# jacarvalho/mpd-public

Measured on AMD Instinct MI355X. Metric: denoising-steps/s, higher is better.
Workload: dtype f32; 1 GPU; cfg2: EnvDense2D-RobotPointMass shape, 100 trajectories (1 context(s)) x H=64 x D=4, T=100 (+5) reverse steps, unguided, U-Net dim_mults (1, 2, 4, 8), one plan = one bench step; parallelism=single, denoising_steps_per_plan=105

## Files before the change

### include/mpdx.h

```cpp
#ifndef MPDX_H
#define MPDX_H

#include <stddef.h>
#include <stdint.h>

#ifdef __cplusplus
extern "C" {
#endif

#define MPDX_E_INVALID   (-1)
#define MPDX_E_NOTFOUND  (-2)
#define MPDX_E_STATE     (-3)

#define MPDX_MAX_LEVELS 8

typedef struct mpdx_unet mpdx_unet;

typedef struct mpdx_unet_cfg {
    int32_t state_dim;
    int32_t n_support_points;
    int32_t unet_input_dim;
    int32_t n_levels;
    int32_t dim_mults[MPDX_MAX_LEVELS];
    int32_t time_emb_dim;
// ... 165 lines not shown
int mpdx_plan(mpdx_unet* u, const float* packed_dev, const float* timetab_dev, int T, const mpdx_step_coefs* coefs,
              int n_without_noise, float* x, const float* noise, const float* hard_start, const float* hard_goal,
              float* chain, int B, float* ws, const mpdx_guide_params* guide, int n_guide_steps, int t_start_guide,
              uint32_t* guide_flags, int n_per_ctx, uint64_t rng_seed, uint64_t rng_offset, void* stream);

int mpdx_unet_profile(mpdx_unet* u, const float* packed_dev, const float* timetab_dev, int T, const float* x, int t,
                      int B, float* ws, void* stream, int cap, float* ms_out, double* flops_out,
                      const char** names_out, int* n_out);
int mpdx_layer_trace(mpdx_unet* u, const float* packed_dev, const float* timetab_dev, const float* x, int layer, int B, float* ws,
                     void* stream, long long* stamps32);
int mpdx_fused_trace(mpdx_unet* u, const float* packed_dev, const float* timetab_dev, const float* x, int seg, int B,
                     float* ws, void* stream, long long* stamps_out, int cap, int* n_out, int* nops_out);
int mpdx_unet_time_units(mpdx_unet* u, const float* packed_dev, const float* timetab_dev, int T, const float* x, int t, int B,
                         float* ws, void* stream, int unit_first, int unit_last, int reps, float* ms_avg);
int mpdx_unet_time_without(mpdx_unet* u, const float* packed_dev, const float* timetab_dev, int T, const float* x, int t, int B,
                           float* ws, void* stream, unsigned long long skip_mask, int reps, float* ms_avg);
int mpdx_unet_unit_layer(const mpdx_unet* u, int B, int i);
int mpdx_unet_fused_program(const mpdx_unet* u, int seg);
double mpdx_unet_unit_bytes(const mpdx_unet* u, int B, int i);
int mpdx_unet_unit_is_pair(const mpdx_unet* u, int B, int i);
int mpdx_bench_layer(mpdx_unet* u, const float* packed_dev, const float* timetab_dev, const float* x, int layer, int B,
                     float* ws, void* stream, int reps, int dbg, float* ms_per_launch);
int mpdx_unet_layer_tile(const mpdx_unet* u, int i, int B, char* buf, size_t buflen);

#ifdef __cplusplus
}
#endif
#endif
```

### mpd_public_amd/_lib.py

```python
from __future__ import annotations

import ctypes as C
from pathlib import Path

import os as _os

_LIB_PATH = Path(_os.environ["MPDX_LIB"]) if _os.environ.get("MPDX_LIB") else Path(__file__).resolve().parent / "libmpdx.so"
_lib = None

MAX_LEVELS = 8


class UnetCfg(C.Structure):
    _fields_ = [("state_dim", C.c_int32), ("n_support_points", C.c_int32), ("unet_input_dim", C.c_int32),
                ("n_levels", C.c_int32), ("dim_mults", C.c_int32 * MAX_LEVELS), ("time_emb_dim", C.c_int32),
                ("self_attention", C.c_int32)]


class StepCoefs(C.Structure):
    _fields_ = [("sqrt_recip_alphas_cumprod", C.c_float), ("sqrt_recipm1_alphas_cumprod", C.c_float),
                ("posterior_mean_coef1", C.c_float), ("posterior_mean_coef2", C.c_float),
                ("noise_scale", C.c_float), ("noise_std_extra", C.c_float),
                ("predict_epsilon", C.c_int32), ("clip_denoised", C.c_int32), ("ddim_k1", C.c_float), ("ddim_k2", C.c_float),
                ("guide_scale", C.c_float)]
# ... 56 lines not shown
    "mpdx_weighted_loss": (_i, [_vp, _vp, _vp, _vp, _vp, _i, _vp, _i, _i, _i, _vp]),
    "mpdx_plan": (_i, [_vp, _vp, _vp, _i, C.POINTER(StepCoefs), _i, _vp, _vp, _vp, _vp, _vp, _i, _vp,
                        C.POINTER(GuideParams), _i, _i, _vp, _i, C.c_uint64, C.c_uint64, _vp]),
    "mpdx_guide_step": (_i, [C.POINTER(GuideParams), _vp, _vp, _vp, _vp, _vp, _vp, _i, _i, _i, _i, _vp]),
    "mpdx_guide_step_scaled": (_i, [C.POINTER(GuideParams), _vp, _vp, _vp, _vp, _vp, _vp, _i, _i, _i, _i, _f, _vp]),
    "mpdx_guide_time": (_i, [C.POINTER(GuideParams), _vp, _vp, _vp, _i, _i, _i, _i, _i, _vp, C.POINTER(C.c_float)]),
    "mpdx_traj_metrics": (_i, [C.POINTER(GuideParams), _vp, _vp, _i, _i, _i, _i, _vp]),
    "mpdx_traj_metrics_mask": (_i, [C.POINTER(GuideParams), _vp, _vp, _vp, _i, _i, _i, _i, _vp]),
    "mpdx_guide_trace": (_i, [C.POINTER(GuideParams), _vp, _vp, _i, _i, _i, _vp, C.POINTER(C.c_longlong)]),
    "mpdx_absmax": (_i, [_vp, _vp, _i, _i, _i, _i, _vp]),
    "mpdx_sdf_grid_bake": (_i, [C.POINTER(GuideParams), _i, _vp, _vp, C.POINTER(C.c_int * 3), C.POINTER(C.c_float * 3), _f, _vp]),
    "mpdx_unet_profile": (_i, [_vp, _vp, _vp, _i, _vp, _i, _i, _vp, _vp, _i, C.POINTER(C.c_float), C.POINTER(C.c_double),
                                C.POINTER(C.c_char_p), C.POINTER(C.c_int)]),
    "mpdx_layer_trace": (_i, [_vp, _vp, _vp, _vp, _i, _i, _vp, _vp, C.POINTER(C.c_longlong)]),
    "mpdx_fused_trace": (_i, [_vp, _vp, _vp, _vp, _i, _i, _vp, _vp, C.POINTER(C.c_longlong), _i, C.POINTER(C.c_int), C.POINTER(C.c_int)]),
    "mpdx_unet_time_units": (_i, [_vp, _vp, _vp, _i, _vp, _i, _i, _vp, _vp, _i, _i, _i, C.POINTER(C.c_float)]),
    "mpdx_unet_time_without": (_i, [_vp, _vp, _vp, _i, _vp, _i, _i, _vp, _vp, C.c_uint64, _i, C.POINTER(C.c_float)]),
    "mpdx_unet_unit_layer": (_i, [_vp, _i, _i]),
    "mpdx_unet_unit_is_pair": (_i, [_vp, _i, _i]),
    "mpdx_unet_unit_bytes": (C.c_double, [_vp, _i, _i]),
    "mpdx_unet_fused_program": (_i, [_vp, _i]),
    "mpdx_bench_layer": (_i, [_vp, _vp, _vp, _vp, _i, _i, _vp, _vp, _i, _i, C.POINTER(C.c_float)]),
    "mpdx_unet_layer_tile": (_i, [_vp, _i, _i, C.c_char_p, _sz]),
    "mpdx_randn": (_i, [_vp, _sz, C.c_uint64, C.c_uint64, _vp]),
    "mpdx_train_flat_floats": (_sz, [_vp]),
    "mpdx_train_dgrad_pack_floats": (_sz, [_vp]),
    "mpdx_train_workspace_floats": (_sz, [_vp, _i]),
    "mpdx_train_param_offset": (_i, [_vp, _i, C.POINTER(_sz), C.POINTER(_sz)]),
    "mpdx_train_pack": (_i, [_vp, _vp, _vp, _vp, _vp]),
    "mpdx_train_loss_backward": (_i, [_vp, _vp, _vp, _vp, _vp, _vp, _vp, _vp, _vp, _vp, _vp, _vp, _vp, _vp, _i, _i, _i, _i, _f, _vp, _vp, _vp]),
    "mpdx_adam_step": (_i, [_vp, _vp, _vp, _vp, _sz, _f, _f, _f, _f, _i, _f, _vp, _vp]),
    "mpdx_train_draw": (_i, [_vp, C.c_uint64, _vp]),
    "mpdx_ema_update": (_i, [_vp, _vp, _sz, _f, _vp]),
    "mpdx_gpmp_step": (_i, [C.POINTER(GuideParams), C.POINTER(GpmpOpts), _vp, _vp, _vp, _i, _i, _i, _i, _vp]),
    "mpdx_rrt_paths": (_i, [C.POINTER(GuideParams), _vp, _vp, _vp, _vp, _vp, _vp, _vp, _i, _i, _i, _f, _i, _i, _vp]),
    "mpdx_rrt_connect": (_i, [C.POINTER(GuideParams), C.POINTER(RrtOpts), _vp, _vp, _vp, _vp, _vp, _vp, _vp, _i, _vp]),
}


def lib_path() -> Path:
    return _LIB_PATH


class LibraryUnavailable(RuntimeError):
    """libmpdx.so is missing or cannot be loaded on this host (every compute entry point raises it; nothing falls back)"""

# ... 38 lines not shown
```

### mpd_public_amd/csrc/conv_block.hpp

```cpp
#pragma once
#include <hip/hip_runtime.h>
#include <stdint.h>

#include <type_traits>

#if defined(MPDX_LOOP_ABLATION) && !defined(MPDX_DEV_HOOKS)
#define MPDX_DEV_HOOKS 1
#endif
#ifdef MPDX_DEV_HOOKS
#define MPDX_TRACE_PTR(p) (p)
#define MPDX_DBG(a, bits) ((a).dbg & (bits))
#else
#define MPDX_TRACE_PTR(p) ((long long*)nullptr)
#define MPDX_DBG(a, bits) (0)
#endif

namespace mpdx {

typedef float f32x4 __attribute__((ext_vector_type(4)));
typedef float f32x2 __attribute__((ext_vector_type(2)));

enum : int { CONV_S1 = 0, CONV_DOWN = 1, CONV_UPT = 2 };
enum : int { EPI_BIAS = 0, EPI_GN_MISH = 1, EPI_GN_MISH_GEN = 2, EPI_GN_BWD = 3 };

// ... 99 lines not shown
    const float u2 = ((float)(c2 >> 8) + 0.5f) * (1.0f / 16777216.0f), u3 = ((float)(c3 >> 8) + 0.5f) * (1.0f / 16777216.0f);
    const float r0 = sqrtf(-2.0f * logf(u0)), r1 = sqrtf(-2.0f * logf(u2));
    float s0, cs0, s1, cs1;
    sincosf(6.28318530717958647692f * u1, &s0, &cs0);
    sincosf(6.28318530717958647692f * u3, &s1, &cs1);
    z[0] = r0 * cs0; z[1] = r0 * s0; z[2] = r1 * cs1; z[3] = r1 * s1;
}
__device__ __forceinline__ float philox_normal_at(uint64_t seed, uint64_t offset, uint64_t i) {
    float z[4];
    philox_normal4(seed, offset + (i >> 2), z);
    const int c = (int)(i & 3);
    return c == 0 ? z[0] : c == 1 ? z[1] : c == 2 ? z[2] : z[3];
}

template <int MODE, int KS>
struct ConvGeom {
    static constexpr int PAD = (MODE == CONV_S1) ? KS / 2 : 1;
    static constexpr int NTAP = (MODE == CONV_UPT) ? 2 : KS;
    static constexpr int NSLOT = (MODE == CONV_UPT) ? 4 : KS;
};

__host__ __device__ inline int upt_slot_to_k(int slot) { return slot == 0 ? 1 : slot == 1 ? 3 : slot == 2 ? 2 : 0; }

struct GeoAny { static constexpr int L = 0, NC16 = 0, RSPAD = 0; };
template <int NC16_> struct GeoL8 { static constexpr int L = 8, NC16 = NC16_, RSPAD = 8; };
template <int NC16_> struct GeoUp8 { static constexpr int L = 8, NC16 = NC16_, RSPAD = 4; };
constexpr int geo_ilog2(int v) { return v <= 1 ? 0 : 1 + geo_ilog2(v >> 1); }

template <int MODE, int KS, int EPI, int MT, int NT, int WN, int WK, class GEO = GeoAny, int TBRES = -1>
__device__ __forceinline__ void conv_block_body(const ConvArgs& a, const int block_id) {
    using G = ConvGeom<MODE, KS>;
    constexpr bool GK = GEO::L > 0;
    static_assert(!GK || MODE == CONV_S1 || MODE == CONV_UPT, "compile-time geometry: stride-1 and transposed convolutions on 8 input positions");
    constexpr int NWAVE = WN * WK, NTHR = 64 * NWAVE;
    constexpr int MS = MT / 16, NSUB = NT / 16, NSW = NSUB / WN;
    constexpr int PAD = G::PAD, NTAP = G::NTAP, NSLOT = G::NSLOT;
    constexpr int MTP = MT + 4;
    constexpr int MTP4 = MTP / 4;
    static_assert(NSUB % WN == 0, "N split");
    static_assert(MODE != CONV_UPT || (NSW % 2 == 0), "transposed conv pairs even/odd sub-tiles");

    extern __shared__ __attribute__((aligned(16))) float smem[];

    const int tid = threadIdx.x, lane = tid & 63;
    if constexpr (GK) __builtin_assume(tid < NTHR);
    const int wave = __builtin_amdgcn_readfirstlane(tid >> 6);
    const int wn = wave % WN, wk = wave / WN;
    int tr_i = 0;
#define CB_STAMP() do { if (MPDX_TRACE_PTR(a.trace) && tid == 0 && (block_id == 0 || block_id == (int)gridDim.x - 1)) a.trace[(block_id ? 16 : 0) + tr_i] = (long long)__builtin_readcyclecounter(); ++tr_i; } while (0)
    const int n_mt = a.C_out / MT;
    const int mt = block_id % n_mt, nt = block_id / n_mt;
    constexpr int GLO = (MODE == CONV_UPT) ? 2 * GEO::L : GEO::L;
    const int L_in = GK ? GEO::L : a.L_in, L_out = GK ? GLO : a.L_out;
    const int lg_Lin = GK ? geo_ilog2(GEO::L) : a.lg_Lin, lg_Lout = GK ? geo_ilog2(GLO) : a.lg_Lout, lg_c4n = GK ? geo_ilog2(GEO::NC16 * 4) : a.lg_c4n;
    const int spt = NT >> lg_Lout;
    const int s0 = nt * spt;
    const int LP = L_in + 2 * PAD;
    const int RS4 = GK ? (GEO::NC16 * 16 + GEO::RSPAD) / 4 : a.rs >> 2;
    f32x4* const smem4 = (f32x4*)smem;
    const int cin = GK ? GEO::NC16 * 16 : a.c1 + a.c2;
    const int c4n = GK ? GEO::NC16 * 4 : a.cin_pad >> 2;

    CB_STAMP();
    constexpr int NCLS = (MODE == CONV_UPT) ? 2 : 1;
#ifndef MPDX_PF
#define MPDX_PF 2
#endif
    constexpr int PF = MPDX_PF;
    const int nc16 = GK ? GEO::NC16 : a.cin_pad >> 4;
    const int ngroups = nc16 * NTAP;
    const __amdgpu_buffer_rsrc_t wrs = __builtin_amdgcn_make_buffer_rsrc((void*)a.wp, 0, 0x7fffffff, 0x00020000);
    const int wlane = lane * 16;
    const int wtile = (mt * MS) * nc16 * NSLOT * 1024;
    f32x4 af[PF][MS][NCLS];
    auto load_a = [&](int g, f32x4 (&dst)[MS][NCLS]) {
        const int c16 = g / NTAP, ts = g - c16 * NTAP;
#pragma unroll
        for (int m = 0; m < MS; ++m)
#pragma unroll
            for (int p = 0; p < NCLS; ++p) {
                const int slot = (MODE == CONV_UPT) ? (p * 2 + ts) : ts;
                dst[m][p] = __builtin_bit_cast(f32x4, __builtin_amdgcn_raw_buffer_load_b128(wrs, wlane, wtile + ((m * nc16 + c16) * NSLOT + slot) * 1024, 0));
            }
    };
    const int niter = (ngroups + WK - 1) / WK;
    auto ring_g = [&](int it) { const int g = wk + it * WK; return g < ngroups ? g : ngroups - 1; };
    auto ring_init = [&]() {
#pragma unroll
        for (int u = 0; u < PF; ++u) load_a(ring_g(u), af[u]);
    };
#ifdef MPDX_RING_FIRST
    ring_init();
#endif

    if (!MPDX_DBG(a, 1)) {
        const int total = (spt << lg_Lin) << lg_c4n;
        const bool vec_ok = GK ? true : ((a.c1 & 3) == 0) && ((a.c2 & 3) == 0);
        constexpr int SB = 4;
        auto stage_pass = [&](int base, auto vec, auto first) {
            constexpr bool VEC = decltype(vec)::value;
            constexpr bool FIRST = decltype(first)::value;
            f32x4 v[SB];
            int dsto[SB], cc[SB];
            bool ok[SB];
            size_t pos[SB];
#pragma unroll
            for (int u = 0; u < SB; ++u) {
                const int idx = base + u * NTHR;
                const bool in = idx < total;
                const int idc = in ? idx : 0;
                const int rowi = idc >> lg_c4n, c = (idc & (c4n - 1)) << 2;
                const int s = rowi >> lg_Lin, li = rowi & (L_in - 1);
                const int b = s0 + s;
                dsto[u] = in ? (s * LP + li + PAD) * RS4 + (c >> 2) : -1;
                ok[u] = in && b < a.B && c < cin;
                cc[u] = c < cin ? c : 0;
                pos[u] = (size_t)(b < a.B ? b : a.B - 1) * L_in + li;
// ... 24 lines not shown
                }
                if (dsto[u] >= 0) smem4[dsto[u]] = ok[u] ? v[u] : (f32x4){0.f, 0.f, 0.f, 0.f};
            }
        };
        if (vec_ok) {
            stage_pass(tid, std::true_type{}, std::true_type{});
            for (int base = tid + NTHR * SB; base < total; base += NTHR * SB) stage_pass(base, std::true_type{}, std::false_type{});
        } else {
            stage_pass(tid, std::false_type{}, std::true_type{});
            for (int base = tid + NTHR * SB; base < total; base += NTHR * SB) stage_pass(base, std::false_type{}, std::false_type{});
        }
        if (PAD > 0) {
            constexpr int P2 = PAD > 0 ? 2 * PAD : 1;
            const int htot = (spt * P2) << lg_c4n;
            for (int idx = tid; idx < htot; idx += NTHR) {
                const int hr = idx >> lg_c4n, c4 = idx & (c4n - 1);
                const int s = hr / P2, k = hr - s * P2;
                const int lp = (k < PAD) ? k : (L_in + k);
                smem4[(s * LP + lp) * RS4 + c4] = (f32x4){0.f, 0.f, 0.f, 0.f};
            }
        }
    }
#ifndef MPDX_RING_FIRST
    if (MPDX_DBG(a, 1)) ring_init();
#endif
    CB_STAMP();
    __syncthreads();
    CB_STAMP();

    const int j = lane & 15, q = lane >> 4;
    int boff[NSW];
    int npos[NSW];
#pragma unroll
    for (int i = 0; i < NSW; ++i) {
        const int ns = wn * NSW + i;
        if (MODE == CONV_UPT) {
            const int gm = (ns >> 1) * 16 + j;
            const int s = gm >> lg_Lin, m = gm & (L_in - 1);
            boff[i] = (s * LP + m + PAD) * RS4 + q;
            npos[i] = s * L_out + 2 * m + (ns & 1);
        } else {
            const int n = ns * 16 + j;
            const int s = n >> lg_Lout, l = n & (L_out - 1);
            const int r0 = (MODE == CONV_DOWN) ? 2 * l : l;
            boff[i] = (s * LP + r0) * RS4 + q;
            npos[i] = n;
        }
    }

    f32x4 acc[MS][NSW];
#pragma unroll
    for (int m = 0; m < MS; ++m)
#pragma unroll
        for (int i = 0; i < NSW; ++i) acc[m][i] = (f32x4){0.f, 0.f, 0.f, 0.f};

    auto kgroup = [&](const int g, f32x4 (&afu)[MS][NCLS]) {
        const int c16 = g / NTAP, ts = g - c16 * NTAP;
#pragma unroll
        for (int i = 0; i < NSW; ++i) {
            const int p = (MODE == CONV_UPT) ? (i & 1) : 0;
            const int roff = (MODE == CONV_UPT) ? ((ts == 0) ? 0 : (p == 0 ? -1 : 1)) : ts;
#ifdef MPDX_LOOP_ABLATION
            const f32x4 bf = (a.dbg & 32) ? (f32x4){1.f, 2.f, 3.f, 4.f} : smem4[boff[i] + roff * RS4 + c16 * 4];
#else
            const f32x4 bf = smem4[boff[i] + roff * RS4 + c16 * 4];
#endif
#pragma unroll
            for (int e = 0; e < 4; ++e)
#pragma unroll
                for (int m = 0; m < MS; ++m)
                    acc[m][i] = __builtin_amdgcn_mfma_f32_16x16x4f32(afu[m][p][e], bf[e], acc[m][i], 0, 0, 0);
        }
    };
    if constexpr (GK) {
        constexpr int NGR = GEO::NC16 * NTAP;
        constexpr int NIT = (NGR + WK - 1) / WK;
        static_assert(NGR % WK == 0, "GeoL8: the k-groups split evenly over the K-split waves");
        if (!MPDX_DBG(a, 2)) {
#pragma unroll
            for (int it = 0; it < NIT; ++it) {
// ... 11 lines not shown
            if (!(a.dbg & 8)) load_a(ring_g(it0 + u + PF), af[u]);
#else
            load_a(ring_g(it0 + u + PF), af[u]);
#endif
        }
    }

    CB_STAMP();
    __syncthreads();
    CB_STAMP();
    float* red = smem;
#pragma unroll
    for (int m = 0; m < MS; ++m)
#pragma unroll
        for (int i = 0; i < NSW; ++i)
            smem4[(wk * NT + npos[i]) * MTP4 + m * 4 + q] = acc[m][i];
    __syncthreads();
    CB_STAMP();

    if (MPDX_DBG(a, 4)) {
        if (tid == 0 && red[0] == 123.456f) a.dst[0] = red[1];
        return;
    }
    if constexpr (EPI == EPI_GN_MISH_GEN) {
        const int gs = a.gs;
        const int lg_gpt = (MT == 32 ? 5 : 4) - a.lg_gs;
        const int gpt = 1 << lg_gpt;
        const int nreg = spt << lg_gpt;
        const int re = gs << a.lg_Lout;
        const int Lv = (a.Lv_out > 0 && a.Lv_out < L_out) ? a.Lv_out : L_out;
        const float inv_re = 1.0f / (float)(gs * Lv);
        auto region = [&](auto w_, auto nch_, int s, int gl, int b) {
            constexpr int W = decltype(w_)::value, NCH = decltype(nch_)::value;
            float v[NCH][W], tb[NCH][W], rsd[NCH][W], ga[NCH][W], be[NCH][W];
            size_t o[NCH];
            bool ok[NCH];
            float sum = 0.f;
#pragma unroll
            for (int k = 0; k < NCH; ++k) {
                const int e0 = (k * 64 + lane) * W;
                const int l = e0 >> a.lg_gs, c = gl * gs + (e0 & (gs - 1));
                const int n = s * L_out + l, co = mt * MT + c;
                ok[k] = l < Lv;
                o[k] = ((size_t)(b < a.B ? b : 0) * L_out + l) * a.C_out + co;
#pragma unroll
                for (int e = 0; e < W; ++e) {
// ... 250 lines not shown
```

### mpd_public_amd/csrc/host.hpp

```cpp
#pragma once
#include <hip/hip_runtime.h>

#include <algorithm>
#include <cmath>
#include <cstdarg>
#include <cstdio>
#include <cstdlib>
#include <cstring>
#include <mutex>
#include <set>
#include <string>
#include <unordered_map>
#include <vector>

#include "../../include/mpdx.h"
#include "conv_block.hpp"
#include "conv_ws.hpp"
#include "fused_level.hpp"
#include "switches.hpp"
#include "train_types.hpp"

namespace mpdx {

int fail(int code, const char* fmt, ...);
// ... 101 lines not shown
    };
    bool train_ready = false;
    size_t flat_floats = 0, packedT_floats = 0;
    std::vector<TrainLayer> tl;
    std::vector<mpdx::PackDesc> pack_descs_host;
    void* pack_descs_dev = nullptr;
    void* pack_chunks_dev = nullptr;
    size_t n_pack_chunks = 0;
};

namespace mpdx {

int pick_row_stride(int cin_pad, int mode, int L_in, int L_out, int LP);
void choose_tile(const Layer& l, int B, int& MT, int& NT);
bool layer_ksplit(const Layer& l);
int check_ready(const mpdx_unet* u);
unsigned fused_mask(int B);
bool fused_save_variant(const mpdx_unet::Fused& f);
int ensure_fused_streams(mpdx_unet* u, const float* packed, hipStream_t st);
int claim_fused_stream_jobs(mpdx_unet* u, const float* packed, const void** jobs, int* n);
int launch_final_step(const FinalArgs& fa, hipStream_t st);
int launch_conv_layer(const Layer& l, ConvArgs& a, int B, hipStream_t st);
bool pair_tile(const Layer& l1, const Layer& l2, int B, int& MT, int& NT);
int launch_conv_pair(int MT, int NT, const ConvArgs& a1, const ConvArgs& a2, const Layer& l1, const Layer& l2, hipStream_t st);
struct AttnArgs;
const char* attn_unsupported(int C, int L);
int launch_attention(const Layer& l, AttnArgs& a, int B, hipStream_t st);
int launch_weight_stationary(int variant, const Layer& l, ConvArgs& a, const ConvArgs& a2, int B, hipStream_t st);
int launch_fused_args(const mpdx_unet::Fused& f, const FusedArgs& a, int B, hipStream_t st, bool save = false);
int launch_fused_train(const mpdx_unet::Fused& f, const FusedArgs& a, int B, hipStream_t st);
struct NoiseRng;
int launch_guide(const mpdx_guide_params* gp, float* x, float* grad_out, const float* hs, const float* hg, const uint32_t* amax_in,
                 uint32_t* amax_out, int n_per_ctx, int B, int H, int D, hipStream_t st, const float* noise = nullptr, float noise_scale = 0.f,
                 float noise_extra = 0.f, float* chain = nullptr, float guide_scale = 1.0f, const NoiseRng* rng = nullptr);

}
```

### mpd_public_amd/csrc/k_conv.hip

```cpp
#include "host.hpp"

namespace mpdx {

template <int MODE, int KS, int EPI, int MT, int NT, int WN, int WK>
static int launch_conv(const ConvArgs& a, hipStream_t st) {
    const size_t lds = conv_block_lds_bytes<MODE, KS, MT, NT, WK>(a.L_in, a.L_out, a.rs);
    if (lds > 160 * 1024) return fail(MPDX_E_INVALID, "conv tile needs %zu B of LDS", lds);
    auto kern = conv_block_kernel<MODE, KS, EPI, MT, NT, WN, WK>;
    if (lds > 64 * 1024)
        if (int rc = raise_lds_limit((const void*)kern)) return rc;
    const int grid = (a.C_out / MT) * a.n_tiles_n;
    hipLaunchKernelGGL(kern, dim3(grid), dim3(64 * WN * WK), lds, st, a);
    return 0;
}

static bool geo_l8(const Layer& l, const ConvArgs& a) {
    return l.mode == CONV_S1 && l.L_in == 8 && l.L_out == 8 && l.cin_pad == l.c1 + l.c2 && !(l.c1 & 3) && !(l.c2 & 3) && a.rs == l.cin_pad + 8 &&
           (l.cin_pad == 128 || l.cin_pad == 256 || l.cin_pad == 512) && !a.dbg && !(a.Lv_out > 0 && a.Lv_out < l.L_out) &&
           sw::geo();
}
template <int NC16, int MT, int NT, int TBRES>
static int launch_geo_gn(const ConvArgs& a, hipStream_t st) {
    const size_t lds = conv_block_lds_bytes<CONV_S1, 5, MT, NT, 8>(8, 8, NC16 * 16 + 8);
    if (lds > 160 * 1024) return fail(MPDX_E_INVALID, "conv tile needs %zu B of LDS", lds);
    auto kern = conv_block_kernel<CONV_S1, 5, EPI_GN_MISH, MT, NT, 1, 8, GeoL8<NC16>, TBRES>;
    if (lds > 64 * 1024)
        if (int rc = raise_lds_limit((const void*)kern)) return rc;
    hipLaunchKernelGGL(kern, dim3((a.C_out / MT) * a.n_tiles_n), dim3(512), lds, st, a);
    return 0;
}
static int dispatch_geo_gn(const Layer& l, ConvArgs& a, int MT, int NT, hipStream_t st) {
    if (a.tbias && a.res) return -100;
    const int tbres = a.tbias ? 1 : (a.res ? 2 : 0);
#define MPDX_GEO_TILE(nc, mt, nt)                                                              \
    if (l.cin_pad == nc * 16 && MT == mt && NT == nt) {                                        \
        if (tbres == 1) return launch_geo_gn<nc, mt, nt, 1>(a, st);                            \
        if (tbres == 2) return launch_geo_gn<nc, mt, nt, 2>(a, st);                            \
        return launch_geo_gn<nc, mt, nt, 0>(a, st);                                            \
    }
    MPDX_GEO_TILE(16, 32, 32) MPDX_GEO_TILE(16, 32, 64) MPDX_GEO_TILE(16, 32, 16)
    MPDX_GEO_TILE(8, 16, 32) MPDX_GEO_TILE(8, 16, 64) MPDX_GEO_TILE(8, 32, 32) MPDX_GEO_TILE(8, 32, 64)
    MPDX_GEO_TILE(32, 32, 16) MPDX_GEO_TILE(32, 32, 32) MPDX_GEO_TILE(32, 16, 32) MPDX_GEO_TILE(32, 16, 64)
#undef MPDX_GEO_TILE
    return -100;
}

template <int MODE, int KS, int EPI>
static int dispatch_tile(const Layer& l, ConvArgs& a, int B, hipStream_t st) {
    int MT, NT;
    choose_tile(l, B, MT, NT);
    if (l.cout % MT) MT = 16;
    if (l.cout % MT || NT % l.L_out) return fail(MPDX_E_INVALID, "layer %s: no tile for C_out=%d L=%d", l.name.c_str(), l.cout, l.L_out);
    a.n_tiles_n = (int)(((long)B * l.L_out + NT - 1) / NT);
    const bool ksplit = layer_ksplit(l);
    if constexpr (MODE == CONV_S1 && KS == 5 && EPI == EPI_GN_MISH) {
        if (ksplit && geo_l8(l, a)) {
            const int rc = dispatch_geo_gn(l, a, MT, NT, st);
            if (rc != -100) return rc;
        }
    }
#define MPDX_TILE(mt, nt)                                                                        \
// ... 17 lines not shown
#define MPDX_TILE(mt, nt) \
    if (MT == mt && NT == nt) return launch_conv<MODE, KS, EPI, mt, nt, 1, 8>(a, st);
    MPDX_TILE(32, 64) MPDX_TILE(32, 32) MPDX_TILE(16, 64) MPDX_TILE(16, 32) MPDX_TILE(16, 128) MPDX_TILE(32, 128)
    if constexpr (MODE != CONV_UPT) { MPDX_TILE(32, 16) MPDX_TILE(16, 16) }
#undef MPDX_TILE
    return fail(MPDX_E_INVALID, "no instantiation for tile %dx%d", MT, NT);
}

int launch_conv_layer(const Layer& l, ConvArgs& a, int B, hipStream_t st) {
    if (l.mode == CONV_S1 && l.ks == 5 && l.epi == EPI_GN_MISH) {
        const int re = l.gs * l.L_out;
        if ((re != 128 && re != 256) || (a.Lv_out > 0 && a.Lv_out < l.L_out)) return dispatch_tile<CONV_S1, 5, EPI_GN_MISH_GEN>(l, a, B, st);
        return dispatch_tile<CONV_S1, 5, EPI_GN_MISH>(l, a, B, st);
    }
    if (l.mode == CONV_S1 && l.ks == 1 && l.epi == EPI_BIAS) return dispatch_tile_ksplit_only<CONV_S1, 1, EPI_BIAS>(l, a, B, st);
    if (l.mode == CONV_DOWN && l.ks == 3) return dispatch_tile_ksplit_only<CONV_DOWN, 3, EPI_BIAS>(l, a, B, st);
    if (l.mode == CONV_UPT && l.ks == 4) {
        if (l.L_in == 8 && l.L_out == 16 && l.cin_pad == l.c1 && l.c2 == 0 && !(l.c1 & 3) && a.rs == l.cin_pad + 4 && !a.dbg && !a.pre && !a.accum && !a.dst2 &&
            !(a.Lv_out > 0 && a.Lv_out < l.L_out) && sw::geo()) {
            int MT, NT;
            choose_tile(l, B, MT, NT);
            if (l.cout % MT) MT = 16;
            a.n_tiles_n = (int)(((long)B * l.L_out + NT - 1) / NT);
#define MPDX_GEO_UP(nc, mt, nt)                                                                         \
            if (l.cin_pad == nc * 16 && MT == mt && NT == nt) {                                          \
                const size_t lds = conv_block_lds_bytes<CONV_UPT, 4, mt, nt, 8>(8, 16, nc * 16 + 4);     \
                auto kern = conv_block_kernel<CONV_UPT, 4, EPI_BIAS, mt, nt, 1, 8, GeoUp8<nc>>;          \
                if (lds <= 160 * 1024) {                                                                 \
                    if (lds > 64 * 1024)                                                                 \
                        if (int rc = raise_lds_limit((const void*)kern)) return rc;                      \
                    hipLaunchKernelGGL(kern, dim3((a.C_out / mt) * a.n_tiles_n), dim3(512), lds, st, a); \
                    return 0;                                                                            \
                }                                                                                        \
            }
            MPDX_GEO_UP(8, 16, 64) MPDX_GEO_UP(8, 32, 64) MPDX_GEO_UP(8, 16, 32) MPDX_GEO_UP(8, 32, 32)
#undef MPDX_GEO_UP
        }
        return dispatch_tile_ksplit_only<CONV_UPT, 4, EPI_BIAS>(l, a, B, st);
    }
    if (l.mode == CONV_S1 && l.ks == 5 && l.epi == EPI_BIAS) return dispatch_tile_ksplit_only<CONV_S1, 5, EPI_BIAS>(l, a, B, st);
    if (l.mode == CONV_S1 && l.ks == 3 && l.epi == EPI_BIAS) return dispatch_tile_ksplit_only<CONV_S1, 3, EPI_BIAS>(l, a, B, st);
    return fail(MPDX_E_INVALID, "layer %s: unsupported conv (mode %d k %d epi %d)", l.name.c_str(), l.mode, l.ks, l.epi);
}

template <int MT, int NT, class GEO = GeoAny>
static int launch_pair_t(const ConvArgs& a1, const ConvArgs& a2, const Layer& l1, const Layer& l2, hipStream_t st) {
    const size_t lds = std::max(conv_block_lds_bytes<CONV_S1, 5, MT, NT, 8>(l1.L_in, l1.L_out, l1.rs),
                                conv_block_lds_bytes<CONV_S1, 1, MT, NT, 8>(l2.L_in, l2.L_out, l2.rs));
    if (lds > 160 * 1024) return 0;
    auto kern = conv_pair_kernel<MT, NT, GEO>;
    if (lds > 64 * 1024)
        if (raise_lds_limit((const void*)kern)) return -1;
    const int n1 = (a1.C_out / MT) * a1.n_tiles_n, n2 = (a2.C_out / MT) * a2.n_tiles_n;
    hipLaunchKernelGGL(kern, dim3(n1 + n2), dim3(512), lds, st, a1, a2, n1);
    return 1;
}

int launch_conv_pair(int MT, int NT, const ConvArgs& a1, const ConvArgs& a2, const Layer& l1, const Layer& l2, hipStream_t st) {
    if (geo_l8(l1, a1) && geo_l8(l2, a2) && a1.tbias && !a1.res && l2.rs == l1.rs) {
#define MPDX_GEO_PAIR(nc, mt, nt) if (l1.cin_pad == nc * 16 && MT == mt && NT == nt) return launch_pair_t<mt, nt, GeoL8<nc>>(a1, a2, l1, l2, st);
        MPDX_GEO_PAIR(8, 32, 32) MPDX_GEO_PAIR(8, 32, 64) MPDX_GEO_PAIR(8, 32, 16) MPDX_GEO_PAIR(32, 32, 16) MPDX_GEO_PAIR(32, 32, 32) MPDX_GEO_PAIR(32, 16, 32)
#undef MPDX_GEO_PAIR
    }
#define MPDX_PAIR_TILE(mt, nt) if (MT == mt && NT == nt) return launch_pair_t<mt, nt>(a1, a2, l1, l2, st);
    MPDX_PAIR_TILE(32, 64) MPDX_PAIR_TILE(32, 32) MPDX_PAIR_TILE(16, 64) MPDX_PAIR_TILE(16, 32) MPDX_PAIR_TILE(32, 16) MPDX_PAIR_TILE(16, 16)
#undef MPDX_PAIR_TILE
    return fail(MPDX_E_INVALID, "no pair instantiation for tile %dx%d", MT, NT);
}

}
```

### mpd_public_amd/csrc/mpdx.hip

```cpp
#include "host.hpp"
#include "attn.hpp"
#include "loss.hpp"
#include "scene_table.hpp"

namespace mpdx {

static thread_local char g_err[512] = "";
int fail(int code, const char* fmt, ...) {
    va_list ap;
    va_start(ap, fmt);
    vsnprintf(g_err, sizeof(g_err), fmt, ap);
    va_end(ap);
    return code;
}

int raise_lds_limit(const void* kern) {
    static std::mutex mu;
    static std::set<std::pair<int, const void*>> done;
    int dev = 0;
    HIP_TRY(hipGetDevice(&dev));
    std::lock_guard<std::mutex> lock(mu);
    if (done.count({dev, kern})) return 0;
    HIP_TRY(hipFuncSetAttribute(kern, hipFuncAttributeMaxDynamicSharedMemorySize, 160 * 1024));
    done.insert({dev, kern});
// ... 1711 lines not shown
}

int mpdx_unet_layer_tile(const mpdx_unet* u, int i, int B, char* buf, size_t buflen) {
    if (!u || !buf || i < 0 || i >= (int)u->layers.size()) return fail(MPDX_E_INVALID, "bad layer index");
    const Layer& l = u->layers[i];
    if (l.attn) { snprintf(buf, buflen, "attn %dx%d", attn_cols(l.cout, l.L_out) / l.L_out, l.L_out); return 0; }
    int MT, NT;
    ConvArgs dummy;
    memset(&dummy, 0, sizeof(dummy));
    const Layer* l2 = (i + 1 < (int)u->layers.size() && pair_tile(l, u->layers[i + 1], B, MT, NT)) ? &u->layers[i + 1] : nullptr;
    if (const int v = weight_stationary_variant(l, l2, dummy, B, 0)) {
        if (v == 6) snprintf(buf, buflen, "wsp 32x16/2x1+1x1");
        else if (v >= 4) snprintf(buf, buflen, "wsn 16x16/8x1");
        else snprintf(buf, buflen, "ws %dx16/1x8%s", v == 1 ? 32 : 16, v == 3 ? "+1x1" : "");
        return 0;
    }
    choose_tile(l, B, MT, NT);
    if (l.cout % MT) MT = 16;
    const bool ks = layer_ksplit(l);
    snprintf(buf, buflen, "%dx%d/%dx%d", MT, NT, ks ? 1 : NT / 16, ks ? 8 : 8 / (NT / 16));
    return 0;
}

int mpdx_randn(float* out, size_t n, uint64_t seed, uint64_t offset, void* stream) {
    if (!out) return fail(MPDX_E_INVALID, "null argument");
    if (n == 0) return 0;
    const size_t nquad = (n + 3) / 4;
    hipLaunchKernelGGL(randn_kernel, dim3((unsigned)std::min<size_t>((nquad + 255) / 256, 4096)), dim3(256), 0, (hipStream_t)stream, out, n,
                       seed, offset);
    HIP_TRY(hipGetLastError());
    return 0;
}

}
```

Baseline: 5871 denoising-steps/s.

## Specialize 8-position conv kernels on compile-time channel counts and output width

Adds GeoL8C and GeoUp8C geometry variants that bake input channels and output channels into the conv kernel. This lets tile indexing use shifts and masks, and input staging becomes a fixed set of buffer loads with halo zeroing. New specialized epilogues are added for GroupNorm+Mish with a wave-level group reduction, and for plain bias, writing vectors at constant strides. These variants are dispatched for matching single layers, pairs and transposed upsampling layers, and a probe API is added to report which geometry class a layer uses. The cost is more template instantiations and strict shape preconditions.

```diff
diff --git a/include/mpdx.h b/include/mpdx.h
--- a/include/mpdx.h
+++ b/include/mpdx.h
@@ -211,6 +211,7 @@
 int mpdx_bench_layer(mpdx_unet* u, const float* packed_dev, const float* timetab_dev, const float* x, int layer, int B,
                      float* ws, void* stream, int reps, int dbg, float* ms_per_launch);
 int mpdx_unet_layer_tile(const mpdx_unet* u, int i, int B, char* buf, size_t buflen);
+int mpdx_unet_layer_geo(const mpdx_unet* u, int i, int B);
 
 #ifdef __cplusplus
 }
diff --git a/mpd_public_amd/_lib.py b/mpd_public_amd/_lib.py
--- a/mpd_public_amd/_lib.py
+++ b/mpd_public_amd/_lib.py
@@ -102,6 +102,7 @@
     "mpdx_unet_fused_program": (_i, [_vp, _i]),
     "mpdx_bench_layer": (_i, [_vp, _vp, _vp, _vp, _i, _i, _vp, _vp, _i, _i, C.POINTER(C.c_float)]),
     "mpdx_unet_layer_tile": (_i, [_vp, _i, _i, C.c_char_p, _sz]),
+    "mpdx_unet_layer_geo": (_i, [_vp, _i, _i]),
     "mpdx_randn": (_i, [_vp, _sz, C.c_uint64, C.c_uint64, _vp]),
     "mpdx_train_flat_floats": (_sz, [_vp]),
     "mpdx_train_dgrad_pack_floats": (_sz, [_vp]),
diff --git a/mpd_public_amd/csrc/conv_block.hpp b/mpd_public_amd/csrc/conv_block.hpp
--- a/mpd_public_amd/csrc/conv_block.hpp
+++ b/mpd_public_amd/csrc/conv_block.hpp
@@ -145,15 +145,18 @@
 
 __host__ __device__ inline int upt_slot_to_k(int slot) { return slot == 0 ? 1 : slot == 1 ? 3 : slot == 2 ? 2 : 0; }
 
-struct GeoAny { static constexpr int L = 0, NC16 = 0, RSPAD = 0; };
-template <int NC16_> struct GeoL8 { static constexpr int L = 8, NC16 = NC16_, RSPAD = 8; };
-template <int NC16_> struct GeoUp8 { static constexpr int L = 8, NC16 = NC16_, RSPAD = 4; };
+struct GeoAny { static constexpr int L = 0, NC16 = 0, RSPAD = 0, C1 = 0, COUT = 0; };
+template <int NC16_> struct GeoL8 { static constexpr int L = 8, NC16 = NC16_, RSPAD = 8, C1 = 0, COUT = 0; };
+template <int NC16_> struct GeoUp8 { static constexpr int L = 8, NC16 = NC16_, RSPAD = 4, C1 = 0, COUT = 0; };
+template <int NC16_, int C1_, int COUT_> struct GeoL8C { static constexpr int L = 8, NC16 = NC16_, RSPAD = 8, C1 = C1_, COUT = COUT_; };
+template <int NC16_, int COUT_> struct GeoUp8C { static constexpr int L = 8, NC16 = NC16_, RSPAD = 4, C1 = NC16_ * 16, COUT = COUT_; };
 constexpr int geo_ilog2(int v) { return v <= 1 ? 0 : 1 + geo_ilog2(v >> 1); }
 
 template <int MODE, int KS, int EPI, int MT, int NT, int WN, int WK, class GEO = GeoAny, int TBRES = -1>
 __device__ __forceinline__ void conv_block_body(const ConvArgs& a, const int block_id) {
     using G = ConvGeom<MODE, KS>;
     constexpr bool GK = GEO::L > 0;
+    constexpr bool FX = GEO::C1 > 0;
     static_assert(!GK || MODE == CONV_S1 || MODE == CONV_UPT, "compile-time geometry: stride-1 and transposed convolutions on 8 input positions");
     constexpr int NWAVE = WN * WK, NTHR = 64 * NWAVE;
     constexpr int MS = MT / 16, NSUB = NT / 16, NSW = NSUB / WN;
@@ -171,8 +174,14 @@
     const int wn = wave % WN, wk = wave / WN;
     int tr_i = 0;
 #define CB_STAMP() do { if (MPDX_TRACE_PTR(a.trace) && tid == 0 && (block_id == 0 || block_id == (int)gridDim.x - 1)) a.trace[(block_id ? 16 : 0) + tr_i] = (long long)__builtin_readcyclecounter(); ++tr_i; } while (0)
-    const int n_mt = a.C_out / MT;
-    const int mt = block_id % n_mt, nt = block_id / n_mt;
+    int mt, nt;
+    if constexpr (FX) {
+        constexpr int N_MT = GEO::COUT / MT;
+        mt = block_id & (N_MT - 1); nt = block_id >> geo_ilog2(N_MT);
+    } else {
+        const int n_mt = a.C_out / MT;
+        mt = block_id % n_mt; nt = block_id / n_mt;
+    }
     constexpr int GLO = (MODE == CONV_UPT) ? 2 * GEO::L : GEO::L;
     const int L_in = GK ? GEO::L : a.L_in, L_out = GK ? GLO : a.L_out;
     const int lg_Lin = GK ? geo_ilog2(GEO::L) : a.lg_Lin, lg_Lout = GK ? geo_ilog2(GLO) : a.lg_Lout, lg_c4n = GK ? geo_ilog2(GEO::NC16 * 4) : a.lg_c4n;
@@ -191,13 +200,14 @@
 #endif
     constexpr int PF = MPDX_PF;
     const int nc16 = GK ? GEO::NC16 : a.cin_pad >> 4;
+    auto kgroup_chunk = [](int g) { return FX ? (int)((unsigned)g / (unsigned)NTAP) : g / NTAP; };
     const int ngroups = nc16 * NTAP;
     const __amdgpu_buffer_rsrc_t wrs = __builtin_amdgcn_make_buffer_rsrc((void*)a.wp, 0, 0x7fffffff, 0x00020000);
     const int wlane = lane * 16;
     const int wtile = (mt * MS) * nc16 * NSLOT * 1024;
     f32x4 af[PF][MS][NCLS];
     auto load_a = [&](int g, f32x4 (&dst)[MS][NCLS]) {
-        const int c16 = g / NTAP, ts = g - c16 * NTAP;
+        const int c16 = kgroup_chunk(g), ts = g - c16 * NTAP;
 #pragma unroll
         for (int m = 0; m < MS; ++m)
 #pragma unroll
@@ -216,6 +226,62 @@
     ring_init();
 #endif
 
+    int fx_boff[NSW], fx_npos[NSW];
+
+    if constexpr (FX) {
+        constexpr int C4N = GEO::NC16 * 4, LGC = geo_ilog2(C4N), SPT = NT / GLO, RPU = NTHR / C4N;
+        constexpr int NLD = SPT * GEO::L * C4N / NTHR;
+        constexpr int C2 = GEO::NC16 * 16 - GEO::C1;
+        constexpr int LPC = GEO::L + 2 * PAD, RS4C = (GEO::NC16 * 16 + GEO::RSPAD) / 4;
+        static_assert((SPT * GEO::L * C4N) % NTHR == 0 && NLD >= 1, "GeoL8C: every thread issues the same number of staging loads");
+        static_assert(C2 == 0 || (C2 == GEO::C1 && GEO::C1 == 256 && RPU == 4), "GeoL8C: one source, or two of one wave's width (64 float4) each");
+        static_assert(RPU == 4 || RPU % 8 == 0, "GeoL8C: a load of the workgroup covers half a trajectory or whole ones");
+        const float* sp = (C2 > 0 && (wave & 1)) ? a.src2 : a.src1;
+        const __amdgpu_buffer_rsrc_t srs = __builtin_amdgcn_make_buffer_rsrc((void*)(sp + (unsigned)(s0 * (GEO::L * GEO::C1))), 0,
+                                                                             (a.B - s0) * (GEO::L * GEO::C1 * 4), 0x00020000);
+        const int r = tid >> LGC, c4 = tid & (C4N - 1);
+        const int voff = C2 > 0 ? (r * (GEO::C1 / 4) + lane) * 16 : tid * 16;
+        constexpr int VSTEP = C2 > 0 ? RPU * GEO::C1 * 4 : NTHR * 16;
+        f32x4 v[NLD];
+#pragma unroll
+        for (int u = 0; u < NLD; ++u) v[u] = __builtin_bit_cast(f32x4, __builtin_amdgcn_raw_buffer_load_b128(srs, voff + u * VSTEP, 0, 0));
+#ifndef MPDX_RING_FIRST
+        ring_init();
+#endif
+        asm volatile("" ::"s"(a.dst));
+        if constexpr (TBRES == 1) asm volatile("" ::"s"(a.tbias));
+        if constexpr (TBRES == 2) asm volatile("" ::"s"(a.res));
+        const int dbase = ((r >> 3) * LPC + (r & 7) + PAD) * RS4C + c4;
+        __builtin_amdgcn_sched_barrier(0);
+        if constexpr (PAD > 0) {
+            constexpr int P2 = 2 * PAD, HTOT = SPT * P2 * C4N;
+#pragma unroll
+            for (int k = 0; k < (HTOT + NTHR - 1) / NTHR; ++k) {
+                const int idx = tid + k * NTHR;
+                const int hr = idx >> LGC;
+                const int s = hr >> geo_ilog2(P2), kk = hr & (P2 - 1);
+                const int lp = (kk < PAD) ? kk : (GEO::L + kk);
+                if (HTOT % NTHR == 0 || idx < HTOT) smem4[(s * LPC + lp) * RS4C + c4] = (f32x4){0.f, 0.f, 0.f, 0.f};
+            }
+        }
+#pragma unroll
+        for (int i = 0; i < NSW; ++i) {
+            const int ns = wn * NSW + i, jj = lane & 15, qq = lane >> 4;
+            if (MODE == CONV_UPT) {
+                const int gm = (ns >> 1) * 16 + jj;
+                const int s = gm >> 3, m = gm & 7;
+                fx_boff[i] = (s * LPC + m + PAD) * RS4C + qq;
+                fx_npos[i] = s * GLO + 2 * m + (ns & 1);
+            } else {
+                const int n = ns * 16 + jj;
+                fx_boff[i] = ((n >> 3) * LPC + (n & 7)) * RS4C + qq;
+                fx_npos[i] = n;
+            }
+        }
+        __builtin_amdgcn_sched_barrier(0);
+#pragma unroll
+        for (int u = 0; u < NLD; ++u) smem4[dbase + (((u * RPU) >> 3) * LPC + ((u * RPU) & 7)) * RS4C] = v[u];
+    } else
     if (!MPDX_DBG(a, 1)) {
         const int total = (spt << lg_Lin) << lg_c4n;
         const bool vec_ok = GK ? true : ((a.c1 & 3) == 0) && ((a.c2 & 3) == 0);
@@ -286,7 +352,7 @@
         }
     }
 #ifndef MPDX_RING_FIRST
-    if (MPDX_DBG(a, 1)) ring_init();
+    if (!FX && MPDX_DBG(a, 1)) ring_init();
 #endif
     CB_STAMP();
     __syncthreads();
@@ -297,6 +363,7 @@
     int npos[NSW];
 #pragma unroll
     for (int i = 0; i < NSW; ++i) {
+        if constexpr (FX) { boff[i] = fx_boff[i]; npos[i] = fx_npos[i]; continue; }
         const int ns = wn * NSW + i;
         if (MODE == CONV_UPT) {
             const int gm = (ns >> 1) * 16 + j;
@@ -319,7 +386,7 @@
         for (int i = 0; i < NSW; ++i) acc[m][i] = (f32x4){0.f, 0.f, 0.f, 0.f};
 
     auto kgroup = [&](const int g, f32x4 (&afu)[MS][NCLS]) {
-        const int c16 = g / NTAP, ts = g - c16 * NTAP;
+        const int c16 = kgroup_chunk(g), ts = g - c16 * NTAP;
 #pragma unroll
         for (int i = 0; i < NSW; ++i) {
             const int p = (MODE == CONV_UPT) ? (i & 1) : 0;
@@ -377,6 +444,67 @@
         if (tid == 0 && red[0] == 123.456f) a.dst[0] = red[1];
         return;
     }
+    if constexpr (FX && EPI == EPI_GN_MISH) {
+        constexpr int GS = GEO::COUT / 8, LGGS = geo_ilog2(GS), GPT = MT / GS, SPT = NT / GLO, NREG = SPT * GPT, EPL = GS * GLO / 64;
+        static_assert((EPL == 4 || EPL == 2) && GPT >= 1 && (GPT & (GPT - 1)) == 0 && GS * GPT == MT, "GeoL8C: GroupNorm regions of 128 or 256 elements inside the tile");
+        static_assert(TBRES >= 0, "GeoL8C: what follows Mish is known");
+        typedef float vecE __attribute__((ext_vector_type(EPL)));
+        constexpr float inv_re = 1.0f / (float)(64 * EPL);
+#pragma unroll
+        for (int k = 0; k < (NREG + NWAVE - 1) / NWAVE; ++k) {
+            const int r = wave + k * NWAVE;
+            const int s = r >> geo_ilog2(GPT), gl = r & (GPT - 1);
+            const int b = s0 + s;
+            if ((NREG % NWAVE == 0 || r < NREG) && b < a.B) {
+                const int e0 = lane * EPL;
+                const int l = e0 >> LGGS, c = gl * GS + (e0 & (GS - 1));
+                const int n = s * GLO + l, co = mt * MT + c;
+                const unsigned ob = (unsigned)((b * GLO + l) * GEO::COUT + co) * 4u;
+                const vecE bi = *(const vecE*)(a.bias + co);
+                const vecE ga = *(const vecE*)(a.gamma + co), be = *(const vecE*)(a.beta + co);
+                vecE tb = 0.f, rsd = 0.f;
+                if constexpr (TBRES == 1) tb = *(const vecE*)(a.tbias + co);
+                if constexpr (TBRES == 2) rsd = *(const vecE*)((const char*)a.res + ob);
+                __builtin_amdgcn_sched_barrier(0);
+                vecE v = *(const vecE*)(red + n * MTP + c);
+#pragma unroll
+                for (int kk = 1; kk < WK; ++kk) v += *(const vecE*)(red + (kk * NT + n) * MTP + c);
+                v += bi;
+                float sm;
+                if constexpr (EPL == 4) sm = (v[0] + v[1]) + (v[2] + v[3]); else sm = v[0] + v[1];
+                const float mean = wave_sum(sm) * inv_re;
+                const vecE d = v - mean;
+                float sq;
+                if constexpr (EPL == 4) sq = (d[0] * d[0] + d[1] * d[1]) + (d[2] * d[2] + d[3] * d[3]); else sq = d[0] * d[0] + d[1] * d[1];
+                const float var = wave_sum(sq) * inv_re;
+                const float rstd = gn_rstd(var);
+                vecE y;
+#pragma unroll
+                for (int e = 0; e < EPL; ++e) y[e] = mish_nosel(d[e] * rstd * ga[e] + be[e]);
+                if constexpr (TBRES == 1) y += tb;
+                if constexpr (TBRES == 2) y += rsd;
+                *(vecE*)((char*)a.dst + ob) = y;
+            }
+        }
+    } else
+    if constexpr (FX && EPI == EPI_BIAS) {
+        constexpr int M4 = MT / 4, TOT = NT * M4;
+#pragma unroll
+        for (int k = 0; k < (TOT + NTHR - 1) / NTHR; ++k) {
+            const int idx = tid + k * NTHR;
+            if (TOT % NTHR == 0 || idx < TOT) {
+                const int n = idx >> geo_ilog2(M4), c = (idx & (M4 - 1)) * 4;
+                const int s = n >> geo_ilog2(GLO), l = n & (GLO - 1), b = s0 + s;
+                const int co = mt * MT + c;
+                const int ri = n * MTP4 + (c >> 2);
+                f32x4 v = smem4[ri];
+#pragma unroll
+                for (int kk = 1; kk < WK; ++kk) v += smem4[ri + kk * NT * MTP4];
+                v += *(const f32x4*)(a.bias + co);
+                if (b < a.B) *(f32x4*)((char*)a.dst + (unsigned)((b * GLO + l) * GEO::COUT + co) * 4u) = v;
+            }
+        }
+    } else
     if constexpr (EPI == EPI_GN_MISH_GEN) {
         const int gs = a.gs;
         const int lg_gpt = (MT == 32 ? 5 : 4) - a.lg_gs;
diff --git a/mpd_public_amd/csrc/host.hpp b/mpd_public_amd/csrc/host.hpp
--- a/mpd_public_amd/csrc/host.hpp
+++ b/mpd_public_amd/csrc/host.hpp
@@ -147,6 +147,7 @@
 int launch_final_step(const FinalArgs& fa, hipStream_t st);
 int launch_conv_layer(const Layer& l, ConvArgs& a, int B, hipStream_t st);
 bool pair_tile(const Layer& l1, const Layer& l2, int B, int& MT, int& NT);
+int conv_geo_class(const Layer& l, const Layer* l2, ConvArgs a1, ConvArgs a2, int B, int MT, int NT);
 int launch_conv_pair(int MT, int NT, const ConvArgs& a1, const ConvArgs& a2, const Layer& l1, const Layer& l2, hipStream_t st);
 struct AttnArgs;
 const char* attn_unsupported(int C, int L);
diff --git a/mpd_public_amd/csrc/k_conv.hip b/mpd_public_amd/csrc/k_conv.hip
--- a/mpd_public_amd/csrc/k_conv.hip
+++ b/mpd_public_amd/csrc/k_conv.hip
@@ -1,11 +1,20 @@
 #include "host.hpp"
 
 namespace mpdx {
+
+static thread_local bool g_probe = false;
+static thread_local int g_probe_class = -1;
+template <class GEO>
+static bool probe_only() {
+    if (g_probe) g_probe_class = GEO::C1 > 0 ? 2 : (GEO::L > 0 ? 1 : 0);
+    return g_probe;
+}
 
 template <int MODE, int KS, int EPI, int MT, int NT, int WN, int WK>
 static int launch_conv(const ConvArgs& a, hipStream_t st) {
     const size_t lds = conv_block_lds_bytes<MODE, KS, MT, NT, WK>(a.L_in, a.L_out, a.rs);
     if (lds > 160 * 1024) return fail(MPDX_E_INVALID, "conv tile needs %zu B of LDS", lds);
+    if (probe_only<GeoAny>()) return 0;
     auto kern = conv_block_kernel<MODE, KS, EPI, MT, NT, WN, WK>;
     if (lds > 64 * 1024)
         if (int rc = raise_lds_limit((const void*)kern)) return rc;
@@ -19,11 +28,18 @@
            (l.cin_pad == 128 || l.cin_pad == 256 || l.cin_pad == 512) && !a.dbg && !(a.Lv_out > 0 && a.Lv_out < l.L_out) &&
            sw::geo();
 }
-template <int NC16, int MT, int NT, int TBRES>
+static bool geo_consts(const Layer& l, const ConvArgs& a, int c1, int cout) {
+    const size_t lim = (size_t)1 << 31;
+    return !l.pin_nt && l.c1 == c1 && (l.c2 == 0 ? !a.src2 : (l.c2 == c1 && a.src2)) && l.cout == cout && (l.epi != EPI_GN_MISH || l.gs * 8 == cout) &&
+           !a.stuff && !a.decim && !a.pre && !a.accum && !a.dst2 && !a.c_split && !a.tb_stride && a.B > 0 &&
+           (size_t)a.B * l.L_in * l.c1 * 4 < lim && (size_t)a.B * l.L_out * l.cout * 4 < lim;
+}
+template <class GEO, int MT, int NT, int TBRES>
 static int launch_geo_gn(const ConvArgs& a, hipStream_t st) {
-    const size_t lds = conv_block_lds_bytes<CONV_S1, 5, MT, NT, 8>(8, 8, NC16 * 16 + 8);
+    const size_t lds = conv_block_lds_bytes<CONV_S1, 5, MT, NT, 8>(8, 8, GEO::NC16 * 16 + 8);
     if (lds > 160 * 1024) return fail(MPDX_E_INVALID, "conv tile needs %zu B of LDS", lds);
-    auto kern = conv_block_kernel<CONV_S1, 5, EPI_GN_MISH, MT, NT, 1, 8, GeoL8<NC16>, TBRES>;
+    if (probe_only<GEO>()) return 0;
+    auto kern = conv_block_kernel<CONV_S1, 5, EPI_GN_MISH, MT, NT, 1, 8, GEO, TBRES>;
     if (lds > 64 * 1024)
         if (int rc = raise_lds_limit((const void*)kern)) return rc;
     hipLaunchKernelGGL(kern, dim3((a.C_out / MT) * a.n_tiles_n), dim3(512), lds, st, a);
@@ -32,11 +48,19 @@
 static int dispatch_geo_gn(const Layer& l, ConvArgs& a, int MT, int NT, hipStream_t st) {
     if (a.tbias && a.res) return -100;
     const int tbres = a.tbias ? 1 : (a.res ? 2 : 0);
+#define MPDX_GEOC_TILE(nc, c1, cout, mt, nt)                                                               \
+    if (l.cin_pad == nc * 16 && MT == mt && NT == nt && tbres && geo_consts(l, a, c1, cout)) {             \
+        if (tbres == 1) return launch_geo_gn<GeoL8C<nc, c1, cout>, mt, nt, 1>(a, st);                      \
+        return launch_geo_gn<GeoL8C<nc, c1, cout>, mt, nt, 2>(a, st);                                      \
+    }
+    MPDX_GEOC_TILE(16, 256, 256, 32, 16) MPDX_GEOC_TILE(16, 256, 256, 32, 32)
+    MPDX_GEOC_TILE(8, 128, 128, 16, 16) MPDX_GEOC_TILE(8, 128, 128, 16, 32) MPDX_GEOC_TILE(8, 128, 128, 16, 64)
+#undef MPDX_GEOC_TILE
 #define MPDX_GEO_TILE(nc, mt, nt)                                                              \
     if (l.cin_pad == nc * 16 && MT == mt && NT == nt) {                                        \
-        if (tbres == 1) return launch_geo_gn<nc, mt, nt, 1>(a, st);                            \
-        if (tbres == 2) return launch_geo_gn<nc, mt, nt, 2>(a, st);                            \
-        return launch_geo_gn<nc, mt, nt, 0>(a, st);                                            \
+        if (tbres == 1) return launch_geo_gn<GeoL8<nc>, mt, nt, 1>(a, st);                     \
+        if (tbres == 2) return launch_geo_gn<GeoL8<nc>, mt, nt, 2>(a, st);                     \
+        return launch_geo_gn<GeoL8<nc>, mt, nt, 0>(a, st);                                     \
     }
     MPDX_GEO_TILE(16, 32, 32) MPDX_GEO_TILE(16, 32, 64) MPDX_GEO_TILE(16, 32, 16)
     MPDX_GEO_TILE(8, 16, 32) MPDX_GEO_TILE(8, 16, 64) MPDX_GEO_TILE(8, 32, 32) MPDX_GEO_TILE(8, 32, 64)
@@ -100,18 +124,22 @@
             choose_tile(l, B, MT, NT);
             if (l.cout % MT) MT = 16;
             a.n_tiles_n = (int)(((long)B * l.L_out + NT - 1) / NT);
-#define MPDX_GEO_UP(nc, mt, nt)                                                                         \
-            if (l.cin_pad == nc * 16 && MT == mt && NT == nt) {                                          \
+#define MPDX_GEO_UP(nc, mt, nt, GEO, ok)                                                                \
+            if (l.cin_pad == nc * 16 && MT == mt && NT == nt && (ok)) {                                  \
                 const size_t lds = conv_block_lds_bytes<CONV_UPT, 4, mt, nt, 8>(8, 16, nc * 16 + 4);     \
-                auto kern = conv_block_kernel<CONV_UPT, 4, EPI_BIAS, mt, nt, 1, 8, GeoUp8<nc>>;          \
+                auto kern = conv_block_kernel<CONV_UPT, 4, EPI_BIAS, mt, nt, 1, 8, GEO>;                 \
                 if (lds <= 160 * 1024) {                                                                 \
+                    if (probe_only<GEO>()) return 0;                                                     \
                     if (lds > 64 * 1024)                                                                 \
                         if (int rc = raise_lds_limit((const void*)kern)) return rc;                      \
                     hipLaunchKernelGGL(kern, dim3((a.C_out / mt) * a.n_tiles_n), dim3(512), lds, st, a); \
                     return 0;                                                                            \
                 }                                                                                        \
             }
-            MPDX_GEO_UP(8, 16, 64) MPDX_GEO_UP(8, 32, 64) MPDX_GEO_UP(8, 16, 32) MPDX_GEO_UP(8, 32, 32)
+            using Up128 = GeoUp8C<8, 128>;
+            const bool up128 = geo_consts(l, a, 128, 128);
+            MPDX_GEO_UP(8, 16, 32, Up128, up128) MPDX_GEO_UP(8, 16, 64, Up128, up128) MPDX_GEO_UP(8, 32, 64, Up128, up128)
+            MPDX_GEO_UP(8, 16, 64, GeoUp8<8>, true) MPDX_GEO_UP(8, 32, 64, GeoUp8<8>, true) MPDX_GEO_UP(8, 16, 32, GeoUp8<8>, true) MPDX_GEO_UP(8, 32, 32, GeoUp8<8>, true)
 #undef MPDX_GEO_UP
         }
         return dispatch_tile_ksplit_only<CONV_UPT, 4, EPI_BIAS>(l, a, B, st);
@@ -126,6 +154,7 @@
     const size_t lds = std::max(conv_block_lds_bytes<CONV_S1, 5, MT, NT, 8>(l1.L_in, l1.L_out, l1.rs),
                                 conv_block_lds_bytes<CONV_S1, 1, MT, NT, 8>(l2.L_in, l2.L_out, l2.rs));
     if (lds > 160 * 1024) return 0;
+    if (probe_only<GEO>()) return 1;
     auto kern = conv_pair_kernel<MT, NT, GEO>;
     if (lds > 64 * 1024)
         if (raise_lds_limit((const void*)kern)) return -1;
@@ -136,6 +165,12 @@
 
 int launch_conv_pair(int MT, int NT, const ConvArgs& a1, const ConvArgs& a2, const Layer& l1, const Layer& l2, hipStream_t st) {
     if (geo_l8(l1, a1) && geo_l8(l2, a2) && a1.tbias && !a1.res && l2.rs == l1.rs) {
+#define MPDX_GEOC_PAIR(nc, c1, cout, mt, nt)                                                                    \
+        if (l1.cin_pad == nc * 16 && MT == mt && NT == nt && geo_consts(l1, a1, c1, cout) && geo_consts(l2, a2, c1, cout)) \
+            return launch_pair_t<mt, nt, GeoL8C<nc, c1, cout>>(a1, a2, l1, l2, st);
+        MPDX_GEOC_PAIR(8, 128, 256, 32, 16) MPDX_GEOC_PAIR(8, 128, 256, 32, 32) MPDX_GEOC_PAIR(8, 128, 256, 32, 64)
+        MPDX_GEOC_PAIR(32, 256, 128, 16, 16) MPDX_GEOC_PAIR(32, 256, 128, 32, 16)
+#undef MPDX_GEOC_PAIR
 #define MPDX_GEO_PAIR(nc, mt, nt) if (l1.cin_pad == nc * 16 && MT == mt && NT == nt) return launch_pair_t<mt, nt, GeoL8<nc>>(a1, a2, l1, l2, st);
         MPDX_GEO_PAIR(8, 32, 32) MPDX_GEO_PAIR(8, 32, 64) MPDX_GEO_PAIR(8, 32, 16) MPDX_GEO_PAIR(32, 32, 16) MPDX_GEO_PAIR(32, 32, 32) MPDX_GEO_PAIR(32, 16, 32)
 #undef MPDX_GEO_PAIR
@@ -146,4 +181,12 @@
     return fail(MPDX_E_INVALID, "no pair instantiation for tile %dx%d", MT, NT);
 }
 
+int conv_geo_class(const Layer& l, const Layer* l2, ConvArgs a1, ConvArgs a2, int B, int MT, int NT) {
+    g_probe = true;
+    g_probe_class = -1;
+    const int rc = l2 ? launch_conv_pair(MT, NT, a1, a2, l, *l2, nullptr) : launch_conv_layer(l, a1, B, nullptr);
+    g_probe = false;
+    return rc < 0 ? -1 : g_probe_class;
 }
+
+}
diff --git a/mpd_public_amd/csrc/mpdx.hip b/mpd_public_amd/csrc/mpdx.hip
--- a/mpd_public_amd/csrc/mpdx.hip
+++ b/mpd_public_amd/csrc/mpdx.hip
@@ -1757,6 +1757,24 @@
     return 0;
 }
 
+int mpdx_unet_layer_geo(const mpdx_unet* u, int i, int B) {
+    if (!u || i < 0 || i >= (int)u->layers.size() || B < 1) return fail(MPDX_E_INVALID, "bad layer index or batch");
+    const Layer& l = u->layers[i];
+    if (l.attn) return 3;
+    int MT = 0, NT = 0;
+    const Layer* l2 = (i + 1 < (int)u->layers.size() && pair_tile(l, u->layers[i + 1], B, MT, NT)) ? &u->layers[i + 1] : nullptr;
+    const float* const p = (const float*)(uintptr_t)256;
+    ConvArgs a1, a2;
+    memset(&a2, 0, sizeof(a2));
+    if (int rc = make_conv_args(u, l, p, p, p, (float*)(uintptr_t)256, B, 0, a1)) return rc;
+    if (l2)
+        if (int rc = make_conv_args(u, *l2, p, p, p, (float*)(uintptr_t)256, B, 0, a2)) return rc;
+    if (weight_stationary_variant(l, l2, a1, B, 0)) return 3;
+    if (l2) a1.n_tiles_n = a2.n_tiles_n = (int)(((long)B * l.L_out + NT - 1) / NT);
+    const int cls = conv_geo_class(l, l2, a1, a2, B, MT, NT);
+    return cls < 0 ? fail(MPDX_E_INVALID, "layer %s: no kernel for batch %d", l.name.c_str(), B) : cls;
+}
+
 int mpdx_randn(float* out, size_t n, uint64_t seed, uint64_t offset, void* stream) {
     if (!out) return fail(MPDX_E_INVALID, "null argument");
     if (n == 0) return 0;
```

Measured after the change: 6103 denoising-steps/s (median of 6 runs). +4.0%, better.
